# SSTDV-Project/python-fluid-simulation

Measured on AMD Instinct MI355X. Metric: PressureCGSolver3D CG throughput (cells x iterations / s), higher is better.
Workload: dtype f32; 1 GPU; PressureCGSolver3D 256x256x256 synthetic pool scene, fp32 state; cells_per_gpu=16777216, decomposition=single domain, transport=single, step=one CG iteration (apply + 2 dots + x/r/d updates)

## Files before the change

### python-fluid-simulation_amd/csrc/mfs_pcg_apply.h

```cpp
#pragma once
#include "mfs_common.h"
#include "mfs_cg_core.h"

#define MFS_LDS_BARRIER() asm volatile("s_waitcnt lgkmcnt(0)\n\ts_barrier" ::: "memory")

#ifndef MFS_MARCH_MIN_WAVES
#define MFS_MARCH_MIN_WAVES 3
#endif

namespace mfs {

constexpr int kApplyBlock = 256;
constexpr int kXcds = 8;

template <typename T, int VEC>
__device__ __forceinline__ void stencil_vec(T* __restrict__ out_ptr, vec_t<T, VEC> vc, vec_t<T, VEC> vxp,
                                            vec_t<T, VEC> vxm, vec_t<T, VEC> vyp, vec_t<T, VEC> vym,
                                            vec_t<T, VEC> dg, vec_t<T, VEC> cxp, vec_t<T, VEC> cxm,
                                            vec_t<T, VEC> cyp, vec_t<T, VEC> cym, vec_t<T, VEC> czm, double zl,
                                            double zr, double czr, bool first, bool last, bool active, double& acc,
                                            vec_t<T, VEC> czm2) {
  vec_t<T, VEC> o;
#ifdef MFS_APPLY_NATIVE_MATH
  typedef T C;
#else
  typedef double C;
#endif
#pragma unroll
  for (int j = 0; j < VEC; ++j) {
    const C zm = j == 0 ? (C)zl : (C)vc[j == 0 ? 0 : j - 1];
    const C zp = j == VEC - 1 ? (C)zr : (C)vc[j == VEC - 1 ? j : j + 1];
    const C czp = j == VEC - 1 ? (C)czr : (C)czm[j == VEC - 1 ? j : j + 1];
    C val = 0;
    val -= (C)cxp[j] * (C)vxp[j];
    val -= (C)cxm[j] * (C)vxm[j];
    val -= (C)cyp[j] * (C)vyp[j];
    val -= (C)cym[j] * (C)vym[j];
    val -= czp * zp;
    val -= (C)czm2[j] * zm;
    val += (C)dg[j] * (C)vc[j];
    o[j] = (T)val;
    const bool bnd = (first && j == 0) || (last && j == VEC - 1);
    if (active && !bnd) acc += (double)vc[j] * (double)o[j];
  }
  if (!active) return;
  if (!first && !last) {
    vstore<T, VEC>(out_ptr, o);
  } else {
#pragma unroll
    for (int j = 0; j < VEC; ++j) {
      const bool bnd = (first && j == 0) || (last && j == VEC - 1);
      if (!bnd) out_ptr[j] = o[j];
    }
  }
}

struct ApplyArgs {
  int Nx, Ny, Nz, xb, xe, xchunk, xb2, xe2;
  const int* items = nullptr;
  const int* runrem = nullptr;
  const int* count = nullptr;
};

template <typename T, int VEC>
__global__ void __launch_bounds__(kApplyBlock)
k_pcg_apply_direct(const T* __restrict__ v, T* __restrict__ out, const T* __restrict__ diag,
                   const T* __restrict__ cx, const T* __restrict__ cy, const T* __restrict__ cz, ApplyArgs a,
                   double* __restrict__ partial, const double* __restrict__ done_flag) {
  if (done_flag && *done_flag != 0.0) return;
  const int nzv = a.Nz / VEC;
  const int64_t ipp = (int64_t)(a.Ny - 2) * nzv;
  const int n1 = a.xe - a.xb;
  const int np = n1 + (a.xe2 - a.xb2);
  const int nch = min((int)gridDim.x, kXcds);
  const int xcd = blockIdx.x % nch, slot = blockIdx.x / nch;
  const int nblk = (gridDim.x - xcd + nch - 1) / nch;
  const int p0 = (int)((int64_t)np * xcd / nch), p1 = (int)((int64_t)np * (xcd + 1) / nch);
  const int64_t end = (int64_t)p1 * ipp, stride = (int64_t)nblk * kApplyBlock;
  const int64_t sx = (int64_t)a.Ny * a.Nz, sy = a.Nz;
  double acc = 0.0;
  for (int64_t it = (int64_t)p0 * ipp + (int64_t)slot * kApplyBlock + threadIdx.x; it < end; it += stride) {
    const int px = (int)(it / ipp);
    const int rem = (int)(it - (int64_t)px * ipp);
    const int yy = rem / nzv, zv = rem - (rem / nzv) * nzv;
    const int xx = px < n1 ? a.xb + px : a.xb2 + (px - n1);
    const int64_t base = (int64_t)xx * sx + (int64_t)(yy + 1) * sy + (int64_t)zv * VEC;
    const bool first = zv == 0, last = zv == nzv - 1;
    const auto vc = vload<T, VEC>(v + base);
    const double zl = first ? 0.0 : (double)v[base - 1];
    const double zr = last ? 0.0 : (double)v[base + VEC];
    const double czr = last ? 0.0 : (double)cz[base + VEC];
    stencil_vec<T, VEC>(out + base, vc, vload<T, VEC>(v + base + sx), vload<T, VEC>(v + base - sx),
                        vload<T, VEC>(v + base + sy), vload<T, VEC>(v + base - sy), vload<T, VEC>(diag + base),
                        vload<T, VEC>(cx + base + sx), vload<T, VEC>(cx + base), vload<T, VEC>(cy + base + sy),
                        vload<T, VEC>(cy + base), vload<T, VEC>(cz + base), zl, zr, czr, first, last, true, acc,
                        vload<T, VEC>(cz + base));
  }
  const double tot = block_sum<kApplyBlock>(acc);
  if (threadIdx.x == 0) partial[blockIdx.x] = tot;
}


template <typename T, int VEC>
struct CoefVec {
  vec_t<T, VEC> dg, cxm, cxp, cym, cyp, czm, czm2;
  unsigned char cls;
};

template <typename T, int VEC, bool COMP, int NT, bool LOAD_CXM = true, bool ASYM = false>
__device__ __forceinline__ CoefVec<T, VEC> coef_load(const T* __restrict__ diag, const T* __restrict__ cx,
                                                     const T* __restrict__ cy, const T* __restrict__ cz,
                                                     int64_t b, int64_t sx, int Nz, unsigned char cls,
                                                     const T* __restrict__ cz2 = nullptr) {
  CoefVec<T, VEC> c;
  c.cls = cls;
  if (COMP) {
    const T f = cls == kClsRegular ? (T)1 : (T)0, d = cls == kClsRegular ? (T)6 : (T)0;
#pragma unroll
    for (int j = 0; j < VEC; ++j) { c.dg[j] = d; c.cxm[j] = f; c.cxp[j] = f; c.cym[j] = f; c.cyp[j] = f; c.czm[j] = f; c.czm2[j] = f; }
    if (cls == kClsMixed) {
      c.dg = (NT & 1) ? vload_nt<T, VEC>(diag + b) : vload<T, VEC>(diag + b);
      if (LOAD_CXM) c.cxm = vload<T, VEC>(cx + b);
      c.cxp = (NT & 2) ? vload_nt<T, VEC>(cx + b + sx) : vload<T, VEC>(cx + b + sx);
      c.cym = (NT & 4) ? vload_nt<T, VEC>(cy + b) : vload<T, VEC>(cy + b);
      c.cyp = (NT & 4) ? vload_nt<T, VEC>(cy + b + Nz) : vload<T, VEC>(cy + b + Nz);
      c.czm = (NT & 1) ? vload_nt<T, VEC>(cz + b) : vload<T, VEC>(cz + b);
      if (ASYM) c.czm2 = (NT & 1) ? vload_nt<T, VEC>(cz2 + b) : vload<T, VEC>(cz2 + b);
    }
    if (!ASYM) c.czm2 = c.czm;
    return c;
  }
  c.dg = (NT & 1) ? vload_nt<T, VEC>(diag + b) : vload<T, VEC>(diag + b);
  c.cxm = c.dg;
  c.cxp = (NT & 2) ? vload_nt<T, VEC>(cx + b + sx) : vload<T, VEC>(cx + b + sx);
  c.cym = (NT & 4) ? vload_nt<T, VEC>(cy + b) : vload<T, VEC>(cy + b);
  c.cyp = (NT & 4) ? vload_nt<T, VEC>(cy + b + Nz) : vload<T, VEC>(cy + b + Nz);
  c.czm = (NT & 1) ? vload_nt<T, VEC>(cz + b) : vload<T, VEC>(cz + b);
  if (ASYM) c.czm2 = (NT & 1) ? vload_nt<T, VEC>(cz2 + b) : vload<T, VEC>(cz2 + b);
  else c.czm2 = c.czm;
  return c;
}

template <typename T, int VEC>
__global__ void __launch_bounds__(256)
k_pcg_classify(const T* __restrict__ diag, const T* __restrict__ cx, const T* __restrict__ cy,
               const T* __restrict__ cz, int Nx, int Ny, int Nz, unsigned char* __restrict__ cls,
               const T* __restrict__ cz2) {
  const int nzv = Nz / VEC;
  const int64_t nvec = (int64_t)Nx * Ny * nzv;
  const int64_t iv = (int64_t)blockIdx.x * blockDim.x + threadIdx.x;
  if (iv >= nvec) return;
  const int zv = (int)(iv % nzv), y = (int)((iv / nzv) % Ny), x = (int)(iv / ((int64_t)nzv * Ny));
  const int64_t sx = (int64_t)Ny * Nz, b = iv * VEC;
  bool all_zero = true, all_reg = true;
  if (x > 0 && x < Nx - 1 && y > 0 && y < Ny - 1) {
#pragma unroll
    for (int j = 0; j < VEC; ++j) {
      const int z = zv * VEC + j;
      if (z == 0 || z == Nz - 1) continue;
      const int64_t c = b + j;
      const T k[7] = {diag[c], cx[c], cx[c + sx], cy[c], cy[c + Nz], cz2 ? cz2[c] : cz[c], cz[c + 1]};
      bool z0 = true, r1 = k[0] == (T)6;
#pragma unroll
      for (int q = 0; q < 7; ++q) { z0 = z0 && k[q] == (T)0; if (q) r1 = r1 && k[q] == (T)1; }
      if (cz2 && j == 0) { z0 = z0 && cz[c] == (T)0; r1 = r1 && cz[c] == (T)1; }
      all_zero = all_zero && z0;
      all_reg = all_reg && r1;
    }
  }
  cls[iv] = all_zero ? kClsZero : (all_reg ? kClsRegular : kClsMixed);
}

template <typename T, int VEC>
struct RawVec { vec_t<T, VEC> a, b; };

template <typename T, int VEC, bool FUSE>
struct VSrc {
  const T* __restrict__ v;
  const T* __restrict__ r;
  const T* __restrict__ d_old;
  double beta;
  __device__ __forceinline__ RawVec<T, VEC> raw(int64_t off) const {
    RawVec<T, VEC> w;
    if (!FUSE) { w.a = vload<T, VEC>(v + off); w.b = w.a; }
    else { w.a = vload<T, VEC>(r + off); w.b = vload<T, VEC>(d_old + off); }
    return w;
  }
  __device__ __forceinline__ vec_t<T, VEC> fin(const RawVec<T, VEC>& w) const {
    if (!FUSE) return w.a;
    vec_t<T, VEC> o;
#pragma unroll
    for (int j = 0; j < VEC; ++j) o[j] = (T)((double)w.a[j] + beta * (double)w.b[j]);
    return o;
  }
  __device__ __forceinline__ vec_t<T, VEC> ld(int64_t off) const { return fin(raw(off)); }
};

struct BookArgs {
  double* scal;
  double* hist;
  int64_t hist_cap;
  const double* part_rr;
  int npart, par;
};

template <typename T, int VEC, bool LDS, int NT, bool COMP, bool FUSE, int PD, bool ASYM = false, bool XDEF = false,
          bool BOOK = false, bool LMASK = false>
__global__ void __launch_bounds__(kApplyBlock, MFS_MARCH_MIN_WAVES)
k_pcg_apply_march(const T* __restrict__ v, T* __restrict__ out, const T* __restrict__ diag,
                  const T* __restrict__ cx, const T* __restrict__ cy, const T* __restrict__ cz,
                  const unsigned char* __restrict__ cls, ApplyArgs a, double* __restrict__ partial,
                  const double* __restrict__ done_flag, const T* __restrict__ fr, const T* __restrict__ fd_old,
                  T* __restrict__ fd_new, const double* __restrict__ beta_ptr, const T* __restrict__ cz2,
                  T* __restrict__ xdef = nullptr, const double* __restrict__ alpha_ptr = nullptr, BookArgs bk = BookArgs{}) {
  static_assert(!XDEF || FUSE, "the deferred x update rides on the fused direction update");
  static_assert(!LMASK || (COMP && FUSE && PD == 1), "lane-level masking: compressed, fused, prefetch depth 1");
  static_assert(!BOOK || FUSE, "closing the previous iteration rides on the fused direction update");
  static_assert(kApplyBlock == kBlock, "block_total_of is written for kBlock threads");
  double alpha_x = (XDEF && !BOOK) ? *alpha_ptr : 0.0;
  static_assert(!FUSE || LDS, "the fused direction update is implemented on the LDS march");
  double bk_dn = 0.0, bk_delta = 0.0, bk_dq = 0.0, bk_tol2 = 0.0, bk_acc = 0.0;
  bool book_pending = BOOK;
  double beta_v = 0.0;
  if (BOOK) {
    bk_dn = bk.scal[S_DONE]; bk_delta = bk.scal[S_RING + bk.par]; bk_dq = bk.scal[S_DQ]; bk_tol2 = bk.scal[S_TOL2];
    for (int i = threadIdx.x; i < bk.npart; i += kBlock) bk_acc += bk.part_rr[i];
  } else {
    if (done_flag && *done_flag != 0.0) return;
    if (FUSE) beta_v = *beta_ptr;
  }
  VSrc<T, VEC, FUSE> src{v, fr, fd_old, beta_v};
  extern __shared__ __align__(16) unsigned char smem_raw[];
  T* const smem = reinterpret_cast<T*>(smem_raw);
  const int Nz = a.Nz;
  const int nzv = Nz / VEC;
  const int ipp = (a.Ny - 2) * nzv;
  const int tiles = (ipp + kApplyBlock - 1) / kApplyBlock;
  const int n1 = a.xe - a.xb;
  const int np = n1 + (a.xe2 - a.xb2);
  const bool sparse = a.items != nullptr;
  const int64_t total = sparse ? (int64_t)*a.count : (int64_t)tiles * np;

  const int G = gridDim.x;
  const int nch = min(G, kXcds);
  const int xcd = blockIdx.x % nch, slot = blockIdx.x / nch;
  const int per = G / nch, extra = G - per * nch;
  const int seg = xcd * per + min(xcd, extra) + slot;
  const int64_t s0 = total * seg / G, s1 = total * (seg + 1) / G;
  const int64_t sx = (int64_t)a.Ny * Nz;
  const int tid = threadIdx.x, lane = tid & 63;
  const int tile_elems = kApplyBlock * VEC;
  const int buf_elems = tile_elems + 2 * Nz;
  double acc = 0.0;

  auto close_previous = [&]() -> bool {
    book_pending = false;
    __shared__ double s_rr;
    const double t = block_sum<kBlock>(bk_acc);
    if (threadIdx.x == 0) s_rr = t;
    __syncthreads();
    const double rr = s_rr;
    const bool stop = bk_dn != 0.0 || cg_health(bk_dq, rr) != 0 || rr < bk_tol2;
    if (bk_dn == 0.0 && blockIdx.x == 0 && threadIdx.x == 0) cg_book(bk.scal, bk.hist, bk.hist_cap, bk.par, bk_dq, rr);
    src.beta = rr / bk_delta;
    if (XDEF) alpha_x = bk_delta / bk_dq;
    return stop;
  };

  for (int64_t i = s0; i < s1;) {
    const int64_t it_ = sparse ? (int64_t)a.items[i] : i;
    const int tile = (int)(it_ / np);
    const int pl = (int)(it_ - (int64_t)tile * np);
    const int x0 = pl < n1 ? a.xb + pl : a.xb2 + (pl - n1);
    int len = (int)min((int64_t)((pl < n1 ? a.xe : a.xe2) - x0), s1 - i);
    if (sparse) len = min(len, a.runrem[i]);
    if (a.xchunk > 0) len = min(len, a.xchunk);
    const int x1 = x0 + len;
    i += len;
    const int item_raw = tile * kApplyBlock + tid;
    const bool active = item_raw < ipp;
    const int item = active ? item_raw : ipp - 1;
    const int yy = item / nzv, zv = item - yy * nzv;
    const bool first = zv == 0, last = zv == nzv - 1;
    const int64_t m = (int64_t)(yy + 1) * Nz + (int64_t)zv * VEC;
    const int64_t m0 = (int64_t)Nz + (int64_t)tile * tile_elems;
    const int tile_len = min(tile_elems, ipp * VEC - tile * tile_elems);

    int64_t base = (int64_t)x0 * sx + m;
    const RawVec<T, VEC> wm = src.raw(base - sx), wc = src.raw(base), wp = src.raw(base + sx);
    constexpr bool MASK = LMASK;
    const bool mask_on = MASK && sparse;
    unsigned char cls_n = kClsMixed, cls_c = kClsMixed, cls_n2 = kClsMixed;
    if (COMP) {
      cls_c = cls[base / VEC];
      cls_n = cls[(base + (x0 + 1 < x1 ? sx : 0)) / VEC];
      if (MASK) cls_n2 = cls[((int64_t)min(x0 + 2, x1) * sx + m) / VEC];
    }
    RawVec<T, VEC> wh = {};
    const bool h0 = LDS && tid < 2 * nzv;
    if (h0) wh = src.raw((int64_t)x0 * sx + (tid < nzv ? m0 - Nz + tid * VEC : m0 + tile_len + (tid - nzv) * VEC));
    if (BOOK && book_pending) {
      if (close_previous()) return;
    }
    vec_t<T, VEC> vm = src.fin(wm), vc = src.fin(wc), vp = src.fin(wp);
    CoefVec<T, VEC> cc = coef_load<T, VEC, COMP, NT, true, ASYM>(diag, cx, cy, cz, base, sx, Nz, cls_c, cz2);
    if (!COMP) cc.cxm = vload<T, VEC>(cx + base);

    if (LDS) {
      T* b0 = smem;
      if (active) vstore<T, VEC>(b0 + Nz + tid * VEC, vc);
      if (h0) vstore<T, VEC>(b0 + (tid < nzv ? tid * VEC : Nz + tile_len + (tid - nzv) * VEC), src.fin(wh));
      for (int s = tid + kApplyBlock; s < 2 * nzv; s += kApplyBlock) {
        const bool lo = s < nzv;
        const int j = lo ? s : s - nzv;
        vstore<T, VEC>(b0 + (lo ? j * VEC : Nz + tile_len + j * VEC),
                       src.ld((int64_t)x0 * sx + (lo ? m0 - Nz + j * VEC : m0 + tile_len + j * VEC)));
      }
      MFS_LDS_BARRIER();
    }
    const bool hact = LDS && tid < 2 * nzv;
    const bool hlow = tid < nzv;
    const int64_t hg = hlow ? m0 - Nz + (int64_t)tid * VEC : m0 + tile_len + (int64_t)(tid - nzv) * VEC;
    const int hl = hlow ? tid * VEC : Nz + tile_len + (tid - nzv) * VEC;
    RawVec<T, VEC> Q[PD > 1 ? PD - 1 : 1], H[PD];
#pragma unroll
    for (int k = 0; k < PD - 1; ++k) Q[k] = src.raw((int64_t)min(x0 + 2 + k, x1) * sx + m);
#pragma unroll
    for (int k = 0; k < PD; ++k) {
      H[k] = RawVec<T, VEC>{};
      if (hact) H[k] = src.raw((int64_t)min(x0 + 1 + k, x1) * sx + hg);
    }

    for (int x = x0; x < x1; ++x) {
      const bool more = x + 1 < x1;
      const int cur = (x - x0) & 1;
      const int64_t nb = base + sx;
      const int64_t nn = more ? nb : base;
      const int64_t n2 = more ? nb + sx : nb;
      const bool dead_c = mask_on && cc.cls == kClsDead;
      RawVec<T, VEC> qn = {};
      if (!(mask_on && cls_n2 == kClsDead)) qn = src.raw((int64_t)min(x + 1 + PD, x1) * sx + m);
      vec_t<T, VEC> xo = {}, dxo = {};
      if (XDEF && !dead_c) { xo = vload_nt<T, VEC>(xdef + base); dxo = vload<T, VEC>(fd_old + base); }
      CoefVec<T, VEC> cn = coef_load<T, VEC, COMP, NT, false, ASYM>(diag, cx, cy, cz, nn, sx, Nz, more ? cls_n : cc.cls, cz2);
      cn.cxm = cc.cxp;
      unsigned char cls_nn = kClsMixed;
      if (COMP) cls_nn = MASK ? cls[((int64_t)min(x + 3, x1) * sx + m) / VEC] : cls[n2 / VEC];
      RawVec<T, VEC> hn = {};
      if (hact) hn = src.raw((int64_t)min(x + 1 + PD, x1) * sx + hg);
      vec_t<T, VEC> vym, vyp;
      double zl, zr;
      if (LDS) {
        const T* bc = smem + cur * buf_elems;
        vym = vload<T, VEC>(bc + tid * VEC);
        vyp = vload<T, VEC>(bc + 2 * Nz + tid * VEC);
        zl = (double)bc[Nz + tid * VEC - 1];
        zr = (double)bc[Nz + tid * VEC + VEC];
      } else {
        vym = vload<T, VEC>(v + base - Nz);
        vyp = vload<T, VEC>(v + base + Nz);
        const T l = __shfl_up(vc[VEC - 1], 1, 64), r = __shfl_down(vc[0], 1, 64);
        zl = (double)((lane == 0 && !first) ? v[base - 1] : l);
        zr = (double)((lane == 63 && !last) ? v[base + VEC] : r);
      }
      const T czs = __shfl_down(cc.czm[0], 1, 64);
      const double czr = (double)((lane == 63 && !last) ? cz[base + VEC] : czs);
      stencil_vec<T, VEC>(out + base, vc, vp, vm, vyp, vym, cc.dg, cc.cxp, cc.cxm, cc.cyp, cc.cym, cc.czm, zl, zr, czr,
                          first, last, active && !dead_c, acc, cc.czm2);
      if (FUSE && active && !dead_c) vstore<T, VEC>(fd_new + base, vc);
      if (XDEF && active && !dead_c) {
#pragma unroll
        for (int j = 0; j < VEC; ++j) xo[j] = (T)((double)xo[j] + alpha_x * (double)dxo[j]);
        vstore_nt<T, VEC>(xdef + base, xo);
      }
      if (more) {
        if (LDS) {
          T* bn = smem + (cur ^ 1) * buf_elems;
          if (active) vstore<T, VEC>(bn + Nz + tid * VEC, vp);
          if (hact) vstore<T, VEC>(bn + hl, src.fin(H[0]));
          for (int s = tid + kApplyBlock; s < 2 * nzv; s += kApplyBlock) {
            const bool lo = s < nzv;
            const int j = lo ? s : s - nzv;
            vstore<T, VEC>(bn + (lo ? j * VEC : Nz + tile_len + j * VEC),
                           src.ld((int64_t)(x + 1) * sx + (lo ? m0 - Nz + j * VEC : m0 + tile_len + j * VEC)));
          }
          MFS_LDS_BARRIER();
        }
        vm = vc; vc = vp; vp = src.fin(PD == 1 ? qn : Q[0]); cc = cn;
        if (MASK) { cls_n = cls_n2; cls_n2 = cls_nn; } else cls_n = cls_nn;
#pragma unroll
        for (int k = 0; k + 1 < PD - 1; ++k) Q[k] = Q[k + 1];
        if (PD > 1) Q[PD - 2] = qn;
#pragma unroll
        for (int k = 0; k + 1 < PD; ++k) H[k] = H[k + 1];
        H[PD - 1] = hn;
        base = nb;
      }
    }
    if (LDS) MFS_LDS_BARRIER();
  }
  if (BOOK && book_pending) {
    if (close_previous()) return;
  }
  const double tot = block_sum<kApplyBlock>(acc);
  if (threadIdx.x == 0) partial[blockIdx.x] = tot;
}

}
```

Before: 191,800 Mcells/s.

## Reuse marched source raw values for deferred x update instead of reloading fd_old

The deferred x += alpha*d update no longer loads the old direction from fd_old. It reuses the raw source vectors already streamed through the x-march register pipeline (wc, wp, and the prefetched plane two ahead). The update is shifted two planes ahead so it matches the raw values available in the prefetch queue. This removes one full-field read per cell per iteration, at the cost of more complex ownership and boundary logic, and it depends on the raw source buffer equalling the old direction.

```diff
diff --git a/python-fluid-simulation_amd/csrc/mfs_pcg_apply.h b/python-fluid-simulation_amd/csrc/mfs_pcg_apply.h
--- a/python-fluid-simulation_amd/csrc/mfs_pcg_apply.h
+++ b/python-fluid-simulation_amd/csrc/mfs_pcg_apply.h
@@ -299,10 +299,27 @@
     RawVec<T, VEC> wh = {};
     const bool h0 = LDS && tid < 2 * nzv;
     if (h0) wh = src.raw((int64_t)x0 * sx + (tid < nzv ? m0 - Nz + tid * VEC : m0 + tile_len + (tid - nzv) * VEC));
+    const bool xown_c = XDEF && !(mask_on && cls_c == kClsDead);
+    const bool xown_n = XDEF && x0 + 1 < x1 && !(mask_on && cls_n == kClsDead);
+    vec_t<T, VEC> xo_c = {}, xo_n = {};
+    if (xown_c) xo_c = vload_nt<T, VEC>(xdef + base);
+    if (xown_n) xo_n = vload_nt<T, VEC>(xdef + base + sx);
     if (BOOK && book_pending) {
       if (close_previous()) return;
     }
     vec_t<T, VEC> vm = src.fin(wm), vc = src.fin(wc), vp = src.fin(wp);
+    if (XDEF && active) {
+      if (xown_c) {
+#pragma unroll
+        for (int j = 0; j < VEC; ++j) xo_c[j] = (T)((double)xo_c[j] + alpha_x * (double)wc.b[j]);
+        vstore_nt<T, VEC>(xdef + base, xo_c);
+      }
+      if (xown_n) {
+#pragma unroll
+        for (int j = 0; j < VEC; ++j) xo_n[j] = (T)((double)xo_n[j] + alpha_x * (double)wp.b[j]);
+        vstore_nt<T, VEC>(xdef + base + sx, xo_n);
+      }
+    }
     CoefVec<T, VEC> cc = coef_load<T, VEC, COMP, NT, true, ASYM>(diag, cx, cy, cz, base, sx, Nz, cls_c, cz2);
     if (!COMP) cc.cxm = vload<T, VEC>(cx + base);
 
@@ -340,8 +357,9 @@
       const bool dead_c = mask_on && cc.cls == kClsDead;
       RawVec<T, VEC> qn = {};
       if (!(mask_on && cls_n2 == kClsDead)) qn = src.raw((int64_t)min(x + 1 + PD, x1) * sx + m);
-      vec_t<T, VEC> xo = {}, dxo = {};
-      if (XDEF && !dead_c) { xo = vload_nt<T, VEC>(xdef + base); dxo = vload<T, VEC>(fd_old + base); }
+      const bool xown = XDEF && x + 2 < x1 && !(mask_on && cls_n2 == kClsDead);
+      vec_t<T, VEC> xo = {};
+      if (xown) xo = vload_nt<T, VEC>(xdef + base + 2 * sx);
       CoefVec<T, VEC> cn = coef_load<T, VEC, COMP, NT, false, ASYM>(diag, cx, cy, cz, nn, sx, Nz, more ? cls_n : cc.cls, cz2);
       cn.cxm = cc.cxp;
       unsigned char cls_nn = kClsMixed;
@@ -368,11 +386,6 @@
       stencil_vec<T, VEC>(out + base, vc, vp, vm, vyp, vym, cc.dg, cc.cxp, cc.cxm, cc.cyp, cc.cym, cc.czm, zl, zr, czr,
                           first, last, active && !dead_c, acc, cc.czm2);
       if (FUSE && active && !dead_c) vstore<T, VEC>(fd_new + base, vc);
-      if (XDEF && active && !dead_c) {
-#pragma unroll
-        for (int j = 0; j < VEC; ++j) xo[j] = (T)((double)xo[j] + alpha_x * (double)dxo[j]);
-        vstore_nt<T, VEC>(xdef + base, xo);
-      }
       if (more) {
         if (LDS) {
           T* bn = smem + (cur ^ 1) * buf_elems;
@@ -386,7 +399,13 @@
           }
           MFS_LDS_BARRIER();
         }
-        vm = vc; vc = vp; vp = src.fin(PD == 1 ? qn : Q[0]); cc = cn;
+        const RawVec<T, VEC>& wn2 = PD == 1 ? qn : Q[0];
+        vm = vc; vc = vp; vp = src.fin(wn2); cc = cn;
+        if (xown && active) {
+#pragma unroll
+          for (int j = 0; j < VEC; ++j) xo[j] = (T)((double)xo[j] + alpha_x * (double)wn2.b[j]);
+          vstore_nt<T, VEC>(xdef + base + 2 * sx, xo);
+        }
         if (MASK) { cls_n = cls_n2; cls_n2 = cls_nn; } else cls_n = cls_nn;
 #pragma unroll
         for (int k = 0; k + 1 < PD - 1; ++k) Q[k] = Q[k + 1];
```

New measurement: 191,400 Mcells/s. No clear change (-0.2%).
